# princeton-computational-imaging/Neural-Volume-Super-Resolution

Hardware: AMD Instinct MI355X
Metric: rendered rays/sec (64+128 samples) at 800x800 Lego-like view (higher is better)
Workload: dtype f32 as 2 f16 limbs (3 MFMA products, f32 acc); 1 GPU; Blender-'lego'-like 800x800 view, 64 coarse + 128 fine samples, tri-plane decoder (3x800^2x48 + 32^2x48 planes, 4+4x128 MLP), 1 view per GPU per step; partition=view

## Files before the change

include/nvsr.h:

```cpp
#ifndef NVSR_H
#define NVSR_H
#include <stdint.h>

#ifdef __cplusplus
extern "C" {
#endif

typedef void* nvsr_stream_t;

typedef enum {
    NVSR_OK = 0,
    NVSR_ERR_SHAPE = 1,
    NVSR_ERR_LAUNCH = 2,
    NVSR_ERR_NULL = 3,
    NVSR_ERR_ALIGN = 4
} nvsr_status;

#define NVSR_PLANE_CHANNELS 48
#define NVSR_DEC_CHANNELS 128
#define NVSR_DEC_LAYERS 4
#define NVSR_DECODER_NATURAL_FLOATS 130564
#define NVSR_DECODER_PACKED_F32_FLOATS 130576
#define NVSR_DECODER_PACKED_FLOATS 453136
#define NVSR_DECODER_PACKED_BWD_FLOATS 487424

typedef struct nvsr_scene {
    const float* planes[4];
    int32_t ph[4], pw[4];
    float lo[5];
    float range[5];
    float proj[3][6];
} nvsr_scene;

int nvsr_version(void);

#define NVSR_ARITH_INHERIT (-1)
#define NVSR_ARITH_INVALID (-2)
#define NVSR_ARITH_F32 0
#define NVSR_ARITH_F16X2 2
#define NVSR_ARITH_BF16X3 3
#define NVSR_ARITH_DEFAULT NVSR_ARITH_F16X2
int nvsr_get_decoder_arithmetic(void);
int nvsr_set_decoder_arithmetic(int mode);
int nvsr_set_range_flag(uint32_t* device_word);
uint32_t* nvsr_get_range_flag(void);
int nvsr_release_render_scratch(void);
int64_t nvsr_render_scratch_bytes(void);
int nvsr_internal_group_order(const int* trips, int64_t G, int S, int* out, nvsr_stream_t stream);
int nvsr_internal_copy_group_order(int* dst, int64_t G, nvsr_stream_t stream);
int nvsr_internal_live_order(int* live_n, int64_t N, int S, nvsr_stream_t stream);
int nvsr_internal_colour_order_bins(void);
int nvsr_internal_copy_live_counts(int* dst, int64_t N, nvsr_stream_t stream);
int nvsr_internal_point_order(const int* entries, const float* lists, const float* rays, int64_t N, int S, int bands, int* points, int* steps, int* offsets,
                              nvsr_stream_t stream);
int nvsr_internal_point_bands(void);
int nvsr_internal_copy_point_steps(int* dst, int64_t G, nvsr_stream_t stream);
int64_t nvsr_occupancy_words(int G);
int64_t nvsr_occupancy_workspace_floats(int G, int K);
int nvsr_occupancy_build(const nvsr_scene* scene, const float* packed_decoder, int G, int K, float threshold, int dilate, int arithmetic, uint32_t* grid,
                         float* workspace, nvsr_stream_t stream);
int nvsr_render_pass_occupancy_arith(const nvsr_scene* scene, const float* packed_decoder, int64_t N, int S, const float* rays, const float* z, int lindisp,
                                     int white_bkgd, float* rgb, float* disp, float* acc, float* weights, float* depth, const uint32_t* grid, int G, int arithmetic,
                                     nvsr_stream_t stream);
int nvsr_render_rays_occupancy_arith(const nvsr_scene* scene, const float* packed_coarse, const float* packed_fine, int64_t N, int Nc, int Nf,
                                     const float* rays, int lindisp, int white_bkgd, const float* t_rand, const float* u, float* rgb_c, float* disp_c,
                                     float* acc_c, float* rgb_f, float* disp_f, float* acc_f, float* workspace, const uint32_t* grid_coarse, int G_coarse,
                                     const uint32_t* grid_fine, int G_fine, int arithmetic, nvsr_stream_t stream);
int nvsr_internal_occupancy_probes(const nvsr_scene* scene, int G, int K, float* x, nvsr_stream_t stream);
int nvsr_internal_occupancy_cull(const nvsr_scene* scene, int64_t N, int S, const float* rays, const float* z, int lindisp, const uint32_t* grid, int G, int* kept,
                                 int* kept_n, nvsr_stream_t stream);
int nvsr_internal_copy_kept_counts(int* dst, int64_t N, nvsr_stream_t stream);
int nvsr_limb_gemm_probe(int arithmetic, int K, const float* W, const float* X, float* Y, nvsr_stream_t stream);
#define NVSR_CONV_ARITH_DEFAULT NVSR_ARITH_F16X2
int nvsr_get_conv_arithmetic(void);
int nvsr_set_conv_arithmetic(int mode);

int nvsr_plane_to_channel_last(const float* nchw, float* nhwc, int C, int H, int W, nvsr_stream_t stream);
int nvsr_plane_from_channel_last(const float* nhwc, float* nchw, int C, int H, int W, nvsr_stream_t stream);

int nvsr_pack_decoder(const float* natural, float* packed, nvsr_stream_t stream);

int nvsr_get_ray_bundle(int H, int W, double focal_x, double focal_y, const float* c2w, int padding, double offset,
                        float* ro, float* rd, nvsr_stream_t stream);
int nvsr_get_ray_bundle_at(int H, int W, double focal_x, double focal_y, const float* c2w, double offset, int64_t N, const int32_t* row_col,
                           float* ro, float* rd, nvsr_stream_t stream);
int nvsr_sample_pixels(int64_t total, int H, int W, uint64_t key, int64_t first, int64_t n, const float* image, int channels,
                       int32_t* row_col, float* target, nvsr_stream_t stream);
uint64_t nvsr_sample_key(uint64_t seed, uint64_t calls);
int nvsr_sample_pixels_seq(int64_t total, int H, int W, uint64_t* state, int64_t first, int64_t n, const float* image, int channels,
                           int32_t* row_col, float* target, nvsr_stream_t stream);
#define NVSR_MSE_PAIR_MAX_ELEMS (1 << 22)
int nvsr_mse_pair(int64_t n, const float* a, const float* b, const float* target, float* losses, float* g_a, float* g_b, nvsr_stream_t stream);
int nvsr_mse_pair_sum(int64_t n, const float* a, const float* b, const float* target, float* losses3, nvsr_stream_t stream);
int nvsr_mse_pair_backward(int64_t n, const float* a, const float* b, const float* target, const float* scale_a, const float* scale_b, float* g_a,
                           float* g_b, nvsr_stream_t stream);
int nvsr_ndc_rays(int H, int W, double focal, double near_, int64_t N, const float* ro, const float* rd, float* ro_out,
                  float* rd_out, nvsr_stream_t stream);
int nvsr_pack_rays(int64_t N, const float* ro, const float* rd, const float* view_src, double near_, double far_,
                   float* rays, nvsr_stream_t stream);
int nvsr_coarse_z(int64_t N, int Nc, const float* rays, int lindisp, const float* t_rand, float* z, nvsr_stream_t stream);

int nvsr_sample_pdf(int64_t N, int nb, int ns, const float* bins, const float* weights, const float* u, float* samples,
                    nvsr_stream_t stream);
int nvsr_cumprod_exclusive(int64_t N, int n, const float* in, float* out, nvsr_stream_t stream);
int nvsr_cumprod_exclusive_backward(int64_t N, int n, const float* in, const float* out, const float* g_out, float* g_in,
                                    nvsr_stream_t stream);
int nvsr_sort_rows(int64_t N, int n, const float* in, float* out, nvsr_stream_t stream);
int nvsr_importance_resample(int64_t N, int Nc, int Nf, const float* z_coarse, const float* weights, const float* u,
                             float* z_fine, nvsr_stream_t stream);

int nvsr_importance_resample_rays(int64_t N, int Nc, int Nf, const float* rays, int lindisp, const float* weights, const float* u,
                                  float* z_fine, nvsr_stream_t stream);

int nvsr_triplane_decode(const nvsr_scene* scene, const float* packed_decoder, int64_t P, const float* x, float* out,
                         nvsr_stream_t stream);
int nvsr_triplane_decode_arith(const nvsr_scene* scene, const float* packed_decoder, int64_t P, const float* x, float* out, int arithmetic,
                               nvsr_stream_t stream);

int nvsr_composite(int64_t N, int S, const float* raw, const float* z, const float* rd, const float* noise, int white_bkgd,
                   float* rgb, float* disp, float* acc, float* weights, float* depth, nvsr_stream_t stream);

int nvsr_composite_mip(int64_t N, int S, const float* raw, const float* z, const float* rd, const float* noise, int white_bkgd,
                       float* rgb, float* disp, float* acc, float* weights , float* depth ,
                       nvsr_stream_t stream);
int nvsr_composite_rays(int64_t N, int S, const float* raw, const float* z, const float* rays, const float* noise, int white_bkgd,
                        float* rgb, float* disp, float* acc, float* weights, float* depth, nvsr_stream_t stream);

int nvsr_render_pass(const nvsr_scene* scene, const float* packed_decoder, int64_t N, int S, const float* rays, const float* z,
                     const float* noise, int white_bkgd, float* rgb, float* disp, float* acc, float* weights, float* depth,
                     nvsr_stream_t stream);

int nvsr_decode_rays(const nvsr_scene* scene, const float* packed_decoder, int64_t N, int S, const float* rays, const float* z,
                     float* raw, nvsr_stream_t stream);

#define NVSR_FUSED_MIN_RAYS 65536
int64_t nvsr_fused_min_rays(void);
int64_t nvsr_render_workspace_floats(int64_t N, int Nc, int Nf);
int nvsr_render_rays(const nvsr_scene* scene, const float* packed_coarse, const float* packed_fine, int64_t N, int Nc, int Nf,
// ... 245 lines not shown
```

neural-volume-super-resolution_amd/capi.py:

```python
import ctypes as C
import os

import torch

from .build import LIB_PATH as _DEFAULT_LIB_PATH

LIB_PATH = os.environ.get("NVSR_HIP_LIB", _DEFAULT_LIB_PATH)

PLANE_CHANNELS = 48
DEC_CHANNELS = 128
DECODER_NATURAL_FLOATS = 130564
DECODER_PACKED_FLOATS = 453136
DECODER_PACKED_BWD_FLOATS = 487424
MIP_NERF_NATURAL_FLOATS = 81092
MIP_NERF_RECORD_FLOATS = 767
MIP_NERF_GRAD_RECORD_FLOATS = 708
PE_NERF_NATURAL_FLOATS = 81476
PE_NERF_RECORD_FLOATS = 770
PE_NERF_GRAD_RECORD_FLOATS = 708
MSE_PAIR_MAX_ELEMS = 1 << 22

_STATUS = {1: "NVSR_ERR_SHAPE (argument out of the supported range)", 2: "NVSR_ERR_LAUNCH (kernel launch failed)",
           3: "NVSR_ERR_NULL (required pointer is NULL)", 4: "NVSR_ERR_ALIGN (pointer not 16-byte aligned)"}

# ... 59 lines not shown
    "nvsr_cumprod_exclusive_backward": ([_i64, _i, _vp, _vp, _vp, _vp, _vp], _i),
    "nvsr_importance_resample": ([_i64, _i, _i, _vp, _vp, _vp, _vp, _vp], _i),
    "nvsr_importance_resample_rays": ([_i64, _i, _i, _vp, _i, _vp, _vp, _vp, _vp], _i),
    "nvsr_triplane_decode": ([C.POINTER(Scene), _vp, _i64, _vp, _vp, _vp], _i),
    "nvsr_triplane_decode_arith": ([C.POINTER(Scene), _vp, _i64, _vp, _vp, _i, _vp], _i),
    "nvsr_composite": ([_i64, _i, _vp, _vp, _vp, _vp, _i, _vp, _vp, _vp, _vp, _vp, _vp], _i),
    "nvsr_composite_rays": ([_i64, _i, _vp, _vp, _vp, _vp, _i, _vp, _vp, _vp, _vp, _vp, _vp], _i),
    "nvsr_composite_mip": ([_i64, _i, _vp, _vp, _vp, _vp, _i, _vp, _vp, _vp, _vp, _vp, _vp], _i),
    "nvsr_render_pass": ([C.POINTER(Scene), _vp, _i64, _i, _vp, _vp, _vp, _i, _vp, _vp, _vp, _vp, _vp, _vp], _i),
    "nvsr_decode_rays": ([C.POINTER(Scene), _vp, _i64, _i, _vp, _vp, _vp, _vp], _i),
    "nvsr_render_workspace_floats": ([_i64, _i, _i], _i64),
    "nvsr_render_rays": ([C.POINTER(Scene), _vp, _vp, _i64, _i, _i, _vp, _i, _i, _vp, _vp, _vp, _vp, _vp, _vp, _vp, _vp, _vp,
                          _vp, _vp, _vp], _i),
}
PACK_ALL_ARITHMETICS = -3
_fp = C.POINTER(C.c_float)
_ip = C.POINTER(C.c_int)
_PROTOS_OPTIONAL = {
    "nvsr_conv3x3_packed_floats": ([_i, _i], _i64),
    "nvsr_pack_conv3x3": ([_vp, _i, _i, _vp, _vp], _i),
    "nvsr_conv3x3": ([_vp, _i, _i, _i, _vp, _i, _i, _vp, _vp, _vp], _i),
    "nvsr_edsr_natural_floats": ([_i, _i, _i, _i, _i], _i64),
    "nvsr_edsr_packed_floats": ([_i, _i, _i, _i, _i], _i64),
    "nvsr_pack_edsr": ([_vp, _i, _i, _i, _i, _i, _vp, _vp], _i),
    "nvsr_pack_edsr_arith": ([_vp, _i, _i, _i, _i, _i, _vp, _i, _vp], _i),
    "nvsr_edsr_out_size": ([_i, _i, _i, _i, _ip, _ip], _i),
    "nvsr_edsr_workspace_floats": ([_i, _i, _i, _i, _i], _i64),
    "nvsr_edsr_forward": ([_vp, _i, _i, _i, _vp, _i, _i, _i, _i, _vp, _vp, _vp], _i),
    "nvsr_planes_sr_workspace_floats": ([_i, _i, _i, _i, _i, _i, _i, _fp], _i64),
    "nvsr_planes_sr": ([_vp, _i, _i, _i, _vp, _i, _i, _i, _i, _i, _fp, _vp, _vp, _vp, _vp, _vp], _i),
    "nvsr_render_pass_ex": ([C.POINTER(Scene), _vp, _i64, _i, _vp, _vp, _vp, _i, _vp, _vp, _vp, _vp, _vp, _vp, _vp], _i),
    "nvsr_pack_decoder_bwd": ([_vp, _vp, _vp], _i),
    "nvsr_composite_backward": ([_i64, _i, _vp, _vp, _vp, _vp, _i, _vp, _vp, _vp, _vp], _i),
    "nvsr_composite_backward_mip": ([_i64, _i, _vp, _vp, _vp, _vp, _i, _vp, _vp, _vp, _vp], _i),
    "nvsr_composite_backward_depth": ([_i64, _i, _vp, _vp, _vp, _vp, _i, _vp, _vp, _vp, _i, _vp, _vp], _i),
    "nvsr_composite_backward_rays": ([_i64, _i, _vp, _vp, _vp, _vp, _i, _vp, _vp, _vp, _i, _vp, _vp], _i),
    "nvsr_render_pass_backward": ([C.POINTER(Scene), _vp, _vp, _i64, _i, _vp, _vp, _vp, C.POINTER(C.c_void_p), _vp], _i),
    "nvsr_decode_rays_ex": ([C.POINTER(Scene), _vp, _i64, _i, _vp, _vp, _vp, _vp, _vp, _vp], _i),
    "nvsr_render_pass_backward_gates": ([C.POINTER(Scene), _vp, _vp, _i64, _i, _vp, _vp, _vp, _vp, C.POINTER(C.c_void_p), _vp, _vp, _vp], _i),
    "nvsr_view_grad_workspace_floats": ([_i64, _i], _i64),
    "nvsr_decoder_record_floats": ([_i64, _i], _i64),
    "nvsr_render_pass_backward_ex": ([C.POINTER(Scene), _vp, _vp, _i64, _i, _vp, _vp, _vp, C.POINTER(C.c_void_p), _vp, _vp, _vp], _i),
    "nvsr_decoder_weight_grad": ([_i64, _i, _vp, _vp, _vp], _i),
    "nvsr_edsr_forward_batch": ([_vp, _i, _i, _i, _i, _vp, _i, _i, _i, _i, _vp, _vp, _vp], _i),
    "nvsr_planes_sr_batch": ([C.POINTER(C.c_void_p), _i, _i, _i, _i, _vp, _i, _i, _i, _i, _i, _fp, _vp, _vp, C.POINTER(C.c_void_p), _vp, _vp], _i),
    "nvsr_pack_conv3x3_dgrad": ([_vp, _i, _i, _vp, _vp], _i),
    "nvsr_conv3x3_dgrad": ([_vp, _i, _i, _i, _vp, _i, _vp, _vp], _i),
    "nvsr_conv3x3_wgrad_workspace_floats": ([_i, _i, _i, _i], _i64),
    "nvsr_conv3x3_wgrad": ([_vp, _vp, _i, _i, _i, _i, C.c_float, _vp, _vp, _vp], _i),
    "nvsr_edsr_acts_floats": ([_i, _i, _i, _i, _i, _i, _i], _i64),
    "nvsr_edsr_forward_train": ([_vp, _i, _i, _i, _vp, _i, _i, _i, _i, _vp, _vp, _vp], _i),
    "nvsr_edsr_packed_dgrad_floats": ([_i, _i, _i, _i, _i], _i64),
    "nvsr_pack_edsr_dgrad": ([_vp, _i, _i, _i, _i, _i, _vp, _vp], _i),
    "nvsr_pack_edsr_dgrad_arith": ([_vp, _i, _i, _i, _i, _i, _vp, _i, _vp], _i),
    "nvsr_edsr_backward_workspace_floats": ([_i, _i, _i, _i, _i, _i, _i], _i64),
    "nvsr_edsr_backward": ([_vp, _i, _i, _i, _vp, _vp, _i, _i, _i, _i, _vp, _vp, _vp, _vp, _vp], _i),
    "nvsr_planes_sr_keep_floats": ([_i, _i, _i, _i, _i, _i, _i, _fp], _i64),
    "nvsr_planes_sr_train": ([_vp, _i, _i, _i, _vp, _i, _i, _i, _i, _i, _fp, _vp, _vp, _vp, _vp, _vp, _vp], _i),
    "nvsr_planes_sr_backward_workspace_floats": ([_i, _i, _i, _i, _i, _i, _i, _fp], _i64),
    "nvsr_planes_sr_backward": ([_i, _i, _i, _vp, _vp, _i, _i, _i, _i, _i, _fp, _vp, _vp, _vp, _vp, _vp, _vp], _i),
    "nvsr_generic_decoder_natural_floats": ([C.POINTER(DecoderGeometry)], _i64),
    "nvsr_generic_decode_workspace_floats": ([C.POINTER(DecoderGeometry), _i64], _i64),
    "nvsr_generic_decode": ([C.POINTER(Scene), C.POINTER(DecoderGeometry), _vp, _i64, _vp, _vp, _vp, _vp], _i),
    "nvsr_generic_decode_backward_workspace_floats": ([C.POINTER(DecoderGeometry), _i64], _i64),
    "nvsr_generic_decode_backward": ([C.POINTER(Scene), C.POINTER(DecoderGeometry), _vp, _i64, _vp, _vp, _vp, _vp, _vp, _vp, _vp, _vp, _vp], _i),
    "nvsr_generic_decoder_natural_floats_ext": ([C.POINTER(DecoderGeometry), _i], _i64),
    "nvsr_generic_decode_workspace_floats_ext": ([C.POINTER(DecoderGeometry), _i, _i64], _i64),
    "nvsr_generic_decode_backward_workspace_floats_ext": ([C.POINTER(DecoderGeometry), _i, _i64], _i64),
    "nvsr_generic_decode_ext": ([C.POINTER(SceneExt), C.POINTER(DecoderGeometry), _vp, _i64, _vp, _vp, _vp, _vp, _vp], _i),
    "nvsr_generic_decode_backward_ext": ([C.POINTER(SceneExt), C.POINTER(DecoderGeometry), _vp, _i64, _vp, _vp, _vp, _vp, C.POINTER(C.c_void_p),
                                          _vp, _vp], _i),
    "nvsr_ray_points": ([_i64, _i, _vp, _vp, _vp, _vp], _i),
    "nvsr_render_shared_workspace_floats": ([_i64, _i, _i], _i64),
    "nvsr_render_rays_shared_arith": ([C.POINTER(Scene), _vp, _i64, _i, _i, _vp, _i, _i, _vp, _vp, _vp, _vp, _vp, _vp, _vp, _vp, _vp, _vp, _vp, _i, _vp], _i),
    "nvsr_shared_merge": ([_i64, _i, _i, _vp, _i, _vp, _vp, _vp, _vp, _vp, _vp], _i),
    "nvsr_release_render_scratch": ([], _i),
    "nvsr_render_scratch_bytes": ([], _i64),
    "nvsr_internal_group_order": ([_vp, _i64, _i, _vp, _vp], _i),
    "nvsr_internal_copy_group_order": ([_vp, _i64, _vp], _i),
    "nvsr_internal_live_order": ([_vp, _i64, _i, _vp], _i),
    "nvsr_internal_colour_order_bins": ([], _i),
    "nvsr_internal_copy_live_counts": ([_vp, _i64, _vp], _i),
    "nvsr_internal_point_bands": ([], _i),
    "nvsr_internal_copy_point_steps": ([_vp, _i64, _vp], _i),
    "nvsr_internal_point_order": ([_vp, _vp, _vp, _i64, _i, _i, _vp, _vp, _vp, _vp], _i),
    "nvsr_occupancy_words": ([_i], _i64),
    "nvsr_occupancy_workspace_floats": ([_i, _i], _i64),
    "nvsr_occupancy_build": ([C.POINTER(Scene), _vp, _i, _i, C.c_float, _i, _i, _vp, _vp, _vp], _i),
    "nvsr_render_pass_occupancy_arith": ([C.POINTER(Scene), _vp, _i64, _i, _vp, _vp, _i, _i, _vp, _vp, _vp, _vp, _vp, _vp, _i, _i, _vp], _i),
    "nvsr_render_rays_occupancy_arith": ([C.POINTER(Scene), _vp, _vp, _i64, _i, _i, _vp, _i, _i, _vp, _vp, _vp, _vp, _vp, _vp, _vp, _vp, _vp, _vp, _i, _vp, _i,
                                          _i, _vp], _i),
    "nvsr_internal_occupancy_probes": ([C.POINTER(Scene), _i, _i, _vp, _vp], _i),
    "nvsr_internal_occupancy_cull": ([C.POINTER(Scene), _i64, _i, _vp, _vp, _i, _vp, _i, _vp, _vp, _vp], _i),
    "nvsr_internal_copy_kept_counts": ([_vp, _i64, _vp], _i),
    "nvsr_set_sr_plane_interp": ([_i], _i),
    "nvsr_get_sr_plane_interp": ([], _i),
    "nvsr_set_sr_align_corners": ([_i], _i),
    "nvsr_get_sr_align_corners": ([], _i),
    "nvsr_render_pass_arith": ([C.POINTER(Scene), _vp, _i64, _i, _vp, _vp, _vp, _i, _vp, _vp, _vp, _vp, _vp, _vp, _i, _vp], _i),
    "nvsr_decode_rays_arith": ([C.POINTER(Scene), _vp, _i64, _i, _vp, _vp, _vp, _vp, _vp, _i, _vp], _i),
    "nvsr_render_rays_arith": ([C.POINTER(Scene), _vp, _vp, _i64, _i, _i, _vp, _i, _i, _vp, _vp, _vp, _vp, _vp, _vp, _vp, _vp, _vp,
                                _vp, _vp, _i, _vp], _i),
    "nvsr_render_pass_backward_gates_arith": ([C.POINTER(Scene), _vp, _vp, _i64, _i, _vp, _vp, _vp, _vp, C.POINTER(C.c_void_p), _vp, _vp, _i, _vp], _i),
    "nvsr_decoder_weight_grad_arith": ([_i64, _i, _vp, _vp, _i, _vp], _i),
    "nvsr_conv3x3_arith": ([_vp, _i, _i, _i, _vp, _i, _i, _vp, _vp, _i, _i, _vp], _i),
    "nvsr_conv3x3_dgrad_arith": ([_vp, _i, _i, _i, _vp, _i, _vp, _i, _i, _vp], _i),
    "nvsr_conv3x3_wgrad_arith": ([_vp, _vp, _i, _i, _i, _i, C.c_float, _vp, _vp, _i, _vp], _i),
    "nvsr_edsr_forward_batch_arith": ([_vp, _i, _i, _i, _i, _vp, _i, _i, _i, _i, _vp, _vp, _i, _vp], _i),
    "nvsr_edsr_forward_train_arith": ([_vp, _i, _i, _i, _vp, _i, _i, _i, _i, _vp, _vp, _i, _vp], _i),
    "nvsr_edsr_backward_arith": ([_vp, _i, _i, _i, _vp, _vp, _i, _i, _i, _i, _vp, _vp, _vp, _vp, _i, _vp], _i),
    "nvsr_planes_sr_arith": ([_vp, _i, _i, _i, _vp, _i, _i, _i, _i, _i, _fp, _vp, _vp, _vp, _vp, _i, _vp], _i),
    "nvsr_planes_sr_batch_arith": ([C.POINTER(C.c_void_p), _i, _i, _i, _i, _vp, _i, _i, _i, _i, _i, _fp, _vp, _vp, C.POINTER(C.c_void_p), _vp, _i, _vp], _i),
    "nvsr_planes_sr_train_arith": ([_vp, _i, _i, _i, _vp, _i, _i, _i, _i, _i, _fp, _vp, _vp, _vp, _vp, _vp, _i, _vp], _i),
    "nvsr_planes_sr_backward_arith": ([_i, _i, _i, _vp, _vp, _i, _i, _i, _i, _i, _fp, _vp, _vp, _vp, _vp, _vp, _i, _vp], _i),
    "nvsr_planes_sr_batch_ex": ([C.POINTER(C.c_void_p), _i, _i, _i, _i, _vp, _i, _i, _i, _i, _i, _fp, _vp, _vp, C.POINTER(C.c_void_p), _vp, _i, _i, _i, _vp], _i),
    "nvsr_planes_sr_batch_keep_floats": ([_i, _i, _i, _i, _i, _i, _i, _i, _fp], _i64),
    "nvsr_planes_sr_batch_workspace_floats": ([_i, _i, _i, _i, _i, _i, _i, _i, _fp], _i64),
    "nvsr_planes_sr_batch_backward_workspace_floats": ([_i, _i, _i, _i, _i, _i, _i, _i, _fp], _i64),
    "nvsr_planes_sr_train_batch_arith": ([C.POINTER(C.c_void_p), _i, _i, _i, _i, _vp, _i, _i, _i, _i, _i, _fp, _vp, _vp, C.POINTER(C.c_void_p), _vp, _vp,
                                          _i, _i, _i, _vp], _i),
    "nvsr_planes_sr_backward_batch_arith": ([_i, _i, _i, _i, _vp, _vp, _i, _i, _i, _i, _i, _fp, _vp, C.POINTER(C.c_void_p), _vp, C.POINTER(C.c_void_p), _vp,
                                             _i, _i, _i, _vp], _i),
    "nvsr_planes_sr_backward_batch_marks": ([_i, _i, _i, _i, _vp, _vp, _i, _i, _i, _i, _i, _fp, _vp, C.POINTER(C.c_void_p), _vp, C.POINTER(C.c_void_p), _vp,
                                             _i, _i, _i, _i, C.POINTER(C.c_int32), C.POINTER(C.c_void_p), _vp], _i),
    "nvsr_positional_encoding": ([_i64, _i, _vp, _i, _i, _vp, _vp], _i),
    "nvsr_flexible_nerf_forward": ([_i64, _vp, _i, _i, _i, _i, _i, _vp, _vp, _vp], _i),
    "nvsr_mip_encode": ([_i64, _i, _vp, _vp, _d, _vp, _vp], _i),
    "nvsr_mip_nerf_forward_arith": ([_i64, _i, _vp, _vp, _d, _vp, _vp, _vp, _i, _vp], _i),
    "nvsr_mip_nerf_backward_arith": ([_i64, _vp, _vp, _vp, _vp, _i, _vp], _i),
    "nvsr_mip_nerf_wgrad_workspace_floats": ([_i64], _i64),
    "nvsr_mip_nerf_weight_grad": ([_i64, _vp, _vp, _vp, _vp, _vp], _i),
    "nvsr_pe_encode": ([_i64, _i, _vp, _vp, _vp, _vp], _i),
    "nvsr_pe_nerf_forward_arith": ([_i64, _i, _vp, _vp, _vp, _vp, _vp, _i, _vp], _i),
    "nvsr_pe_nerf_backward_arith": ([_i64, _vp, _vp, _vp, _vp, _i, _vp], _i),
    "nvsr_pe_nerf_wgrad_workspace_floats": ([_i64], _i64),
    "nvsr_pe_nerf_weight_grad": ([_i64, _vp, _vp, _vp, _vp, _vp], _i),
    "nvsr_render_pass_backward_rows_arith": ([C.POINTER(Scene), _vp, _vp, _i64, _i, _vp, _vp, _vp, _vp, C.POINTER(C.c_void_p), _vp, _vp, _i, _vp], _i),
    "nvsr_view_rows_reduce": ([_i64, _i, _vp, _vp, _vp], _i),
    "nvsr_internal_plane_taps": ([C.POINTER(Scene), _i, _i64, _i, _vp, _vp, _vp, _vp, _vp], _i),
    "nvsr_rows_scatter_workspace_bytes": ([_i64], _i64),
    "nvsr_rows_scatter": ([_i64, _vp, _vp, _vp, _i, _i, _vp, _vp, _i64, _vp], _i),
    "nvsr_decoder_weight_grad_det_workspace_floats": ([_i64, _i], _i64),
    "nvsr_decoder_weight_grad_det_arith": ([_i64, _i, _vp, _vp, _vp, _i, _vp], _i),
    "nvsr_lowrank_planes": ([LowrankPlanesArgs, _vp], _i),
    "nvsr_lowrank_planes_backward": ([LowrankPlanesArgs, _vp], _i),
}

_PROTOS_LAUNCH = {
    "nvsr_render_pass2_launch": ([C.POINTER(Scene), _vp, _i64, _i, _vp, _vp, _vp, _i, _vp, _vp, _vp, _vp, _vp, _vp, _vp], _i),
    "nvsr_render_pass3_launch": ([_i, C.POINTER(Scene), _vp, _i64, _i, _vp, _vp, _vp, _i, _vp, _vp, _vp, _vp, _vp, _vp, _vp], _i),
    "nvsr_render_pass3_coarse_z_launch": ([_i, C.POINTER(Scene), _vp, _i64, _i, _vp, _i, _vp, _i, _vp, _vp, _vp, _vp, _vp, _vp, _vp], _i),
    "nvsr_decode_rays_limb_launch": ([_i, C.POINTER(Scene), _vp, _i64, _i, _vp, _vp, _vp, _vp, _vp, _vp], _i),
    "nvsr_decode_rays_pair_launch": ([C.POINTER(Scene), _vp, _i64, _i, _vp, _vp, _vp, _vp, _vp], _i),
}

_lib = None


ARITHMETIC = {"f32": 0, "f16x2": 2, "bf16x3": 3}
SR_BATCH_MAX = 4
ARITH_INHERIT = -1


def arith_code(mode):
    if mode is None:
        return ARITH_INHERIT
# ... 169 lines not shown
```

neural-volume-super-resolution_amd/csrc/colour_order.hip:

```cpp
#include "colour_order.h"
#include "occupancy.h"
#include "nvsr_internal.h"

#include <cstdlib>
#include <mutex>
#include <vector>

namespace nvsr {

constexpr int SORT_TPB = 1024, SORT_WAVES = SORT_TPB / 64, SORT_ROUNDS = 4, SORT_MAX = SORT_TPB * SORT_ROUNDS;
template <int NKEYS>
__device__ __forceinline__ void counting_sort(const int (&key)[SORT_ROUNDS], int nkeys, int n, int (&start)[SORT_ROUNDS], int (&place)[SORT_ROUNDS],
                                              int (&len)[SORT_ROUNDS]) {
    static_assert(NKEYS <= SORT_TPB, "one thread per key sums the tables");
    __shared__ int cnt_s[NKEYS * SORT_WAVES];
    __shared__ int tot_s[NKEYS], start_s[NKEYS];
    const int wave = threadIdx.x >> 6, lane = threadIdx.x & 63;
    const unsigned long long below = (1ull << lane) - 1ull;
    for (int b = 0; b <= nkeys; ++b) {
        int c = 0;
#pragma unroll
        for (int r = 0; r < SORT_ROUNDS; ++r) c += __popcll(__ballot(key[r] == b));
        if (lane == 0) cnt_s[b * SORT_WAVES + wave] = c;
    }
    __syncthreads();
    if ((int)threadIdx.x <= nkeys) {
        int run = 0;
        for (int w = 0; w < SORT_WAVES; ++w) { const int c = cnt_s[threadIdx.x * SORT_WAVES + w]; cnt_s[threadIdx.x * SORT_WAVES + w] = run; run += c; }
        tot_s[threadIdx.x] = run;
    }
    __syncthreads();
    if ((int)threadIdx.x <= nkeys) {
        int run = 0;
        for (int b = nkeys; b > (int)threadIdx.x; --b) run += tot_s[b];
        start_s[threadIdx.x] = run;
    }
    __syncthreads();
#pragma unroll
    for (int r = 0; r < SORT_ROUNDS; ++r) start[r] = place[r] = len[r] = 0;
    if (wave * (64 * SORT_ROUNDS) >= n) return;
    for (int b = 0; b <= nkeys; ++b) {
        int at = cnt_s[b * SORT_WAVES + wave];
#pragma unroll
        for (int r = 0; r < SORT_ROUNDS; ++r) {
            const unsigned long long m = __ballot(key[r] == b);
            if (key[r] == b) place[r] = at + __popcll(m & below);
            at += __popcll(m);
        }
    }
#pragma unroll
    for (int r = 0; r < SORT_ROUNDS; ++r)
        if (key[r] >= 0) { start[r] = start_s[key[r]]; len[r] = tot_s[key[r]]; }
}

static_assert(ORDER_RAYS == SORT_MAX && SORT_WAVES == ORDER_RAYS / RAYS2 && RAYS2 % 64 == 0, "one block of the order per sort, one wave of it per colour workgroup");
__global__ __launch_bounds__(SORT_TPB) void live_order_kernel(int* __restrict__ live_n, long N, int S, int bins, int* __restrict__ group_trip) {
    __shared__ int out_s[ORDER_RAYS];
    const long block_base = (long)blockIdx.x * ORDER_RAYS;
    const int M = (int)(N - block_base < ORDER_RAYS ? N - block_base : ORDER_RAYS);
    const int wave = threadIdx.x >> 6, lane = threadIdx.x & 63;
    int cnt[SORT_ROUNDS], bin[SORT_ROUNDS];
#pragma unroll
    for (int r = 0; r < SORT_ROUNDS; ++r) {
        const int i = wave * (64 * SORT_ROUNDS) + r * 64 + lane;
        cnt[r] = i < M ? live_n[block_base + i] : 0;
        const int b = (int)(((unsigned)cnt[r] * (unsigned)bins + (unsigned)(S - 1)) / (unsigned)S);
        bin[r] = i < M ? (b < bins ? b : bins) : -1;
    }
    int start[SORT_ROUNDS], place[SORT_ROUNDS], len[SORT_ROUNDS];
    counting_sort<ORDER_BINS + 1>(bin, bins, M, start, place, len);
#pragma unroll
    for (int r = 0; r < SORT_ROUNDS; ++r)
        if (bin[r] >= 0) out_s[start[r] + place[r]] = (cnt[r] << ORDER_SHIFT) | (wave * (64 * SORT_ROUNDS) + r * 64 + lane);
    __syncthreads();
#pragma unroll
    for (int r = 0; r < SORT_ROUNDS; ++r) {
        const int i = threadIdx.x + r * SORT_TPB;
        if (i < M) live_n[block_base + i] = out_s[i];
    }
    if (group_trip && wave * RAYS2 < M) {
        int m = 0;
#pragma unroll
        for (int r = 0; r < RAYS2 / 64; ++r) {
            const int i = wave * RAYS2 + r * 64 + lane;
            if (i < M) m = max(m, out_s[i] >> ORDER_SHIFT);
        }
#pragma unroll
        for (int o = 32; o >= 1; o >>= 1) m = max(m, __shfl_xor(m, o));
        if (lane == 0) group_trip[(long)blockIdx.x * SORT_WAVES + wave] = m;
    }
}

constexpr int GORDER_MAX_G = SORT_MAX, GORDER_MAX_S = 511;
__global__ __launch_bounds__(SORT_TPB) void group_order_kernel(const int* __restrict__ group_trip, int G, int S, int sorted, int* __restrict__ group_slot) {
    if (!sorted || G > GORDER_MAX_G || S > GORDER_MAX_S) {
        const unsigned per = (unsigned)G >> 3, rem = (unsigned)G & 7u;
        for (unsigned r = threadIdx.x; r < (unsigned)G; r += SORT_TPB) {
            const unsigned xcd = r & 7u;
            group_slot[r] = (int)(xcd * per + (xcd < rem ? xcd : rem) + (r >> 3));
        }
        return;
    }
    const int wave = threadIdx.x >> 6, lane = threadIdx.x & 63;
    int key[SORT_ROUNDS];
#pragma unroll
    for (int r = 0; r < SORT_ROUNDS; ++r) {
        const int g = wave * (64 * SORT_ROUNDS) + r * 64 + lane;
        const int t = g < G ? group_trip[g] : 0;
        key[r] = g < G ? (t < 0 ? 0 : t > S ? S : t) : -1;
    }
    int start[SORT_ROUNDS], place[SORT_ROUNDS], len[SORT_ROUNDS];
    counting_sort<GORDER_MAX_S + 1>(key, S, G, start, place, len);
#pragma unroll
    for (int r = 0; r < SORT_ROUNDS; ++r) {
        if (key[r] < 0) continue;
        const int run = len[r], per = run >> 3, rem = run & 7, thr = rem * (per + 1);
        const int j = place[r];
        const int k = j < thr ? j / (per + 1) : rem + (j - thr) / (per ? per : 1);
        const int i = j < thr ? j - k * (per + 1) : (j - thr) - (k - rem) * per;
        group_slot[start[r] + k + 8 * i] = wave * (64 * SORT_ROUNDS) + r * 64 + lane;
    }
}

__global__ __launch_bounds__(RAYS2) void point_order_kernel(const int* __restrict__ live_n, const float* __restrict__ live_z, const float* __restrict__ rays_nf,
                                                            long N, int S, int nb, int* __restrict__ pts, int* __restrict__ steps, int* __restrict__ offs) {
    __shared__ int wsum_s[2][RAYS2 / 64], kmin_s[RAYS2], cnt_s[RAYS2], start_s[RAYS2], stage_s[RAYS2];
    const int j = threadIdx.x, wave = j >> 6, lane = j & 63;
    const long slot0 = (long)blockIdx.x * RAYS2;
    int n = 0;
    long ray = 0;
    if (slot0 + j < N) {
        const int e = live_n[slot0 + j];
        n = e >> ORDER_SHIFT;
        ray = slot0 / ORDER_RAYS * ORDER_RAYS + (e & (ORDER_RAYS - 1));
    }
    const float* lz = live_z + ray * S;
    const float nr = rays_nf ? rays_nf[ray * 11 + 6] : 0.0f, fr = rays_nf ? rays_nf[ray * 11 + 7] : 0.0f;
    auto band_of = [&](int k) -> int {
        const float e = lz[k];
        if (!rays_nf) {
            const long long b = (long long)__float_as_int(e) * nb / S;
            return b < 0 ? 0 : b < nb ? (int)b : nb - 1;
        }
        const float u = __fdiv_rn(__fmul_rn(__fsub_rn(e, nr), (float)nb), __fsub_rn(fr, nr));
        return u >= 0.0f ? (u < (float)nb ? (int)u : nb - 1) : 0;
    };
    auto scan = [&](int c, int buf, int& total) -> int {
        int incl = c;
#pragma unroll
        for (int o = 1; o < 64; o <<= 1) { const int v = __shfl_up(incl, o); if (lane >= o) incl += v; }
        if (lane == 63) wsum_s[buf][wave] = incl;
        __syncthreads();
        int before = 0;
        total = 0;
#pragma unroll
        for (int w = 0; w < RAYS2 / 64; ++w) { const int v = wsum_s[buf][w]; if (w < wave) before += v; total += v; }
        return before + incl - c;
    };
    int* out = pts + (long)blockIdx.x * RAYS2 * S;
    int k = 0, base = 0, nextb = n > 0 ? band_of(0) : nb;
    for (int b = 0; b < nb; ++b) {
        const int k0 = k;
        while (k < n && nextb <= b) { ++k; if (k < n) nextb = max(nextb, band_of(k)); }
        int total;
        const int at = base + scan(k - k0, b & 1, total);
        for (int i = k0; i < k; ++i) out[at + (i - k0)] = (j << 24) | i;
        base += total;
    }
    const int nsteps = (base + RAYS2 - 1) / RAYS2;
    if (base + j < nsteps * RAYS2) out[base + j] = POINT_NONE;
    if (j == 0) { steps[blockIdx.x] = nsteps; offs[blockIdx.x] = (int)blockIdx.x * S; }
    __syncthreads();
    for (int t = 0; t < nsteps; ++t) {
        const int e = out[t * RAYS2 + j];
        const bool valid = e != POINT_NONE;
        const int sl = (int)((unsigned)e >> 24), kk = e & 0xffffff;
        kmin_s[j] = 0x7fffffff; cnt_s[j] = 0;
        __syncthreads();
        if (valid) { atomicMin(&kmin_s[sl], kk); atomicAdd(&cnt_s[sl], 1); }
        __syncthreads();
        int total;
        start_s[j] = scan(cnt_s[j], 0, total);
        __syncthreads();
        stage_s[valid ? start_s[sl] + (kk - kmin_s[sl]) : j] = e;
        __syncthreads();
        out[t * RAYS2 + j] = stage_s[j];
    }
}

namespace {
enum { LISTS, GROUP, POINTS, VIEWS, KEPT, KEPT_GROUP, N_BUFFERS };
struct Buffer { void* p; size_t bytes; };
struct Launch { int64_t N; int* n; int* steps; int64_t kept_N; int* kept; };
struct Scratch { int device; hipStream_t stream; Buffer buf[N_BUFFERS]; Launch last; };
std::mutex g_live_mutex;
std::vector<Scratch> g_live;

Scratch* find_scratch(int device, hipStream_t stream) {
    for (Scratch& c : g_live)
        if (c.device == device && c.stream == stream) return &c;
    return nullptr;
}

bool grow(Scratch& e, int which, size_t bytes) {
    Buffer& b = e.buf[which];
    if (b.bytes >= bytes) return true;
    if (b.p) (void)hipFree(b.p);
    b = Buffer{};
    e.last = Launch{};
    void* p = nullptr;
    if (hipMalloc(&p, bytes) != hipSuccess) { (void)hipGetLastError(); return false; }
    b = Buffer{p, bytes};
    return true;
}

int64_t groups_of(int64_t N) { return (N + RAYS2 - 1) / RAYS2; }

template <class Pick>
int copy_left_behind(int* dst, int64_t ints, nvsr_stream_t stream, Pick pick) {
    if (!dst) return NVSR_ERR_NULL;
    int device = 0;
    if (hipGetDevice(&device) != hipSuccess) return NVSR_ERR_LAUNCH;
    const int* src = nullptr;
    {
        std::lock_guard<std::mutex> lock(g_live_mutex);
        const Scratch* c = find_scratch(device, (hipStream_t)stream);
        if (c) src = pick(*c);
    }
    if (!src) return NVSR_ERR_SHAPE;
    return hipMemcpyAsync(dst, src, (size_t)ints * sizeof(int), hipMemcpyDefault, (hipStream_t)stream) == hipSuccess ? NVSR_OK : NVSR_ERR_LAUNCH;
}

bool env_starts(const char* name, char c) {
    const char* e = getenv(name);
    return e && e[0] == c;
}
void launch_live_order(int* live_n, int64_t N, int S, int bins, int* group_trip, hipStream_t stream) {
    hipLaunchKernelGGL(live_order_kernel, dim3((unsigned)((N + ORDER_RAYS - 1) / ORDER_RAYS)), dim3(SORT_TPB), 0, stream, live_n, (long)N, S, bins, group_trip);
}
void launch_group_order(const int* group_trip, int64_t G, int S, int* group_slot, hipStream_t stream) {
    const int sorted = !env_starts("NVSR_COLOUR_GROUP_ORDER", '0');
    hipLaunchKernelGGL(group_order_kernel, dim3(1), dim3(SORT_TPB), 0, stream, group_trip, (int)G, S, sorted, group_slot);
}
void launch_point_order(const int* live_n, const float* live_z, const float* rays_nf, int64_t N, int S, int nb, int* pts, int* steps, int* offs, hipStream_t stream) {
    nb = nb < 1 || nb > S ? S : nb;
    hipLaunchKernelGGL(point_order_kernel, dim3((unsigned)groups_of(N)), dim3(RAYS2), 0, stream, live_n, live_z, rays_nf, (long)N, S, nb, pts, steps, offs);
}
}

PassRoute acquire_pass_scratch(int64_t N, int S, hipStream_t stream, bool raw_out, bool want_kept, bool launch, LiveLists& live, KeptLists& kept) {
    bool declines = raw_out || S < 1 || S >= ORDER_MAX_S || env_starts("NVSR_RENDER_ONE_PHASE", '1');
    if (!declines) {
        hipStreamCaptureStatus cap = hipStreamCaptureStatusNone;
        if (hipStreamIsCapturing(stream, &cap) != hipSuccess || cap != hipStreamCaptureStatusNone) { (void)hipGetLastError(); declines = true; }
    }
    if (declines && !want_kept) return PassRoute::Fused;
    int device = 0;
    if (hipGetDevice(&device) != hipSuccess) return PassRoute::Fused;
    const size_t rows = (size_t)N * (size_t)S, G = (size_t)groups_of(N);
    std::lock_guard<std::mutex> lock(g_live_mutex);
    Scratch* e = find_scratch(device, stream);
    if (e && want_kept) { e->last.kept_N = 0; e->last.kept = nullptr; }
    if (declines) return PassRoute::Fused;
    if (!e) {
        g_live.emplace_back();
        e = &g_live.back();
        e->device = device; e->stream = stream;
    }
    if (!grow(*e, GROUP, 2 * G * sizeof(int)) || !grow(*e, LISTS, (2 * rows + (size_t)N) * sizeof(float)) || !e->buf[LISTS].p) return PassRoute::Fused;
    live = LiveLists{};
    live.z = static_cast<float*>(e->buf[LISTS].p);
    live.w = live.z + rows;
    live.n = reinterpret_cast<int*>(live.w + rows);
    live.slot = static_cast<int*>(e->buf[GROUP].p);
    live.trip = live.slot + G;
    const size_t npts = G * RAYS2 * (size_t)S;
    if (!env_starts("NVSR_COLOUR_POINTS", '0') && G * (size_t)S <= 0x7fffffffu && grow(*e, POINTS, (npts + 2 * G) * sizeof(int)) &&
        grow(*e, VIEWS, G * RAYS2 * POINT_VIEW_FLOATS * sizeof(float))) {
        live.pts = static_cast<int*>(e->buf[POINTS].p);
        live.steps = live.pts + npts;
        live.views = static_cast<float*>(e->buf[VIEWS].p);
    }
    PassRoute route = PassRoute::TwoPhase;
    if (want_kept && grow(*e, KEPT_GROUP, 2 * G * sizeof(int)) && grow(*e, KEPT, (rows + (size_t)N) * sizeof(int))) {
        kept.idx = static_cast<int*>(e->buf[KEPT].p);
        kept.n = kept.idx + rows;
        kept.slot = static_cast<int*>(e->buf[KEPT_GROUP].p);
        kept.trip = kept.slot + G;
        route = PassRoute::Occupancy;
    }
    if (launch) e->last = route == PassRoute::Occupancy ? Launch{N, live.n, live.steps, N, kept.n} : Launch{N, live.n, live.steps, e->last.kept_N, e->last.kept};
    return route;
}

static void launch_orders(int* n, int* trip, int* slot, int64_t N, int S, hipStream_t stream) {
    launch_live_order(n, N, S, env_starts("NVSR_COLOUR_ORDER", '0') ? 0 : ORDER_BINS, trip, stream);
    launch_group_order(trip, groups_of(N), S, slot, stream);
}
void launch_kept_order(const KeptLists& kl, int64_t N, int S, hipStream_t stream) { launch_orders(kl.n, kl.trip, kl.slot, N, S, stream); }
void launch_colour_order(const LiveLists& ll, int64_t N, int S, hipStream_t stream) { launch_orders(ll.n, ll.trip, ll.slot, N, S, stream); }

void launch_point_order(const LiveLists& ll, const float* rays_nf, int64_t N, int S, hipStream_t stream) {
    launch_point_order(ll.n, ll.z, rays_nf, N, S, POINT_BANDS, ll.pts, ll.steps, ll.steps + groups_of(N), stream);
}

}

using namespace nvsr;

extern "C" int nvsr_internal_colour_order_bins(void) { return ORDER_BINS; }
extern "C" int nvsr_internal_live_order(int* live_n, int64_t N, int S, nvsr_stream_t stream) {
    if (!live_n) return NVSR_ERR_NULL;
    if (N < 1 || S < 1 || S >= ORDER_MAX_S || (N + ORDER_RAYS - 1) / ORDER_RAYS > 0x7fffffff) return NVSR_ERR_SHAPE;
    launch_live_order(live_n, N, S, ORDER_BINS, nullptr, (hipStream_t)stream);
    return NVSR_CHECK_LAUNCH();
}
extern "C" int nvsr_internal_copy_live_counts(int* dst, int64_t N, nvsr_stream_t stream) {
    return copy_left_behind(dst, N, stream, [N](const Scratch& c) { return c.last.N == N ? c.last.n : nullptr; });
}
extern "C" int nvsr_internal_group_order(const int* trips, int64_t G, int S, int* out, nvsr_stream_t stream) {
    if (!trips || !out) return NVSR_ERR_NULL;
    if (G < 1 || G > 0x7fffffff || S < 1 || S >= ORDER_MAX_S) return NVSR_ERR_SHAPE;
    launch_group_order(trips, G, S, out, (hipStream_t)stream);
    return NVSR_CHECK_LAUNCH();
}
extern "C" int nvsr_internal_copy_group_order(int* dst, int64_t G, nvsr_stream_t stream) {
    return copy_left_behind(dst, 2 * G, stream, [G](const Scratch& c) { return c.last.n && groups_of(c.last.N) == G ? static_cast<int*>(c.buf[GROUP].p) : nullptr; });
}

extern "C" int nvsr_internal_point_bands(void) { return POINT_BANDS; }
extern "C" int nvsr_internal_point_order(const int* entries, const float* lists, const float* rays, int64_t N, int S, int bands, int* points, int* steps, int* offsets,
                                         nvsr_stream_t stream) {
    if (!entries || !lists || !points || !steps || !offsets) return NVSR_ERR_NULL;
    const int64_t G = (N + RAYS2 - 1) / RAYS2;
    if (N < 1 || S < 1 || S >= ORDER_MAX_S || G * S > 0x7fffffff) return NVSR_ERR_SHAPE;
    launch_point_order(entries, lists, rays, N, S, bands, points, steps, offsets, (hipStream_t)stream);
    return NVSR_CHECK_LAUNCH();
}
extern "C" int nvsr_internal_copy_point_steps(int* dst, int64_t G, nvsr_stream_t stream) {
    return copy_left_behind(dst, G, stream, [G](const Scratch& c) { return c.last.n && groups_of(c.last.N) == G ? c.last.steps : nullptr; });
}

extern "C" int nvsr_internal_copy_kept_counts(int* dst, int64_t N, nvsr_stream_t stream) {
    return copy_left_behind(dst, N, stream, [N](const Scratch& c) { return c.last.kept_N == N ? c.last.kept : nullptr; });
}

extern "C" void nvsr_internal_reserve_render_scratch(int64_t N, int S, nvsr_stream_t stream) {
    LiveLists live;
    KeptLists kept;
    (void)acquire_pass_scratch(N, S, (hipStream_t)stream,  false,  false,  false, live, kept);
}

extern "C" int64_t nvsr_render_scratch_bytes(void) {
    std::lock_guard<std::mutex> lock(g_live_mutex);
    int64_t total = 0;
    for (const Scratch& c : g_live) total += (int64_t)c.buf[LISTS].bytes;
    return total;
}

extern "C" int nvsr_release_render_scratch(void) {
    std::lock_guard<std::mutex> lock(g_live_mutex);
    int prev = 0;
    const bool have_prev = hipGetDevice(&prev) == hipSuccess;
    int rc = NVSR_OK;
    for (const Scratch& c : g_live)
        for (const Buffer& b : c.buf)
            if (b.p && (hipSetDevice(c.device) != hipSuccess || hipFree(b.p) != hipSuccess)) rc = NVSR_ERR_LAUNCH;
    g_live.clear();
    if (have_prev) (void)hipSetDevice(prev);
    return rc;
}
```

Baseline: 8.121 million rays/s.

## Replace looped point-order kernel with single-pass bitmap and band-table counting-sort kernel

Adds a new point_order_kernel for S up to 256. It records each ray's per-band membership in a shared-memory bitmap, builds a per-band, per-wave count table with atomics, and scans it with DPP wave prefix sums. Each thread then places its points directly into 256-wide output steps, reading live_z as float4 when aligned. The old iterative kernel stays as a fallback for larger S. This aims to cut the repeated per-step passes and synchronisations of the loop kernel, but adds complex shared-memory bookkeeping and a larger shared footprint.

New measurement: 8.178 million rays/s (median of 6 runs). About the same (+0.7%).

```diff
diff --git a/include/nvsr.h b/include/nvsr.h
--- a/include/nvsr.h
+++ b/include/nvsr.h
@@ -54,6 +54,7 @@
 int nvsr_internal_point_order(const int* entries, const float* lists, const float* rays, int64_t N, int S, int bands, int* points, int* steps, int* offsets,
                               nvsr_stream_t stream);
 int nvsr_internal_point_bands(void);
+int nvsr_internal_point_order_max_s(void);
 int nvsr_internal_copy_point_steps(int* dst, int64_t G, nvsr_stream_t stream);
 int64_t nvsr_occupancy_words(int G);
 int64_t nvsr_occupancy_workspace_floats(int G, int K);
diff --git a/neural-volume-super-resolution_amd/capi.py b/neural-volume-super-resolution_amd/capi.py
--- a/neural-volume-super-resolution_amd/capi.py
+++ b/neural-volume-super-resolution_amd/capi.py
@@ -165,6 +165,7 @@
     "nvsr_internal_colour_order_bins": ([], _i),
     "nvsr_internal_copy_live_counts": ([_vp, _i64, _vp], _i),
     "nvsr_internal_point_bands": ([], _i),
+    "nvsr_internal_point_order_max_s": ([], _i),
     "nvsr_internal_copy_point_steps": ([_vp, _i64, _vp], _i),
     "nvsr_internal_point_order": ([_vp, _vp, _vp, _i64, _i, _i, _vp, _vp, _vp, _vp], _i),
     "nvsr_occupancy_words": ([_i], _i64),
diff --git a/neural-volume-super-resolution_amd/csrc/colour_order.hip b/neural-volume-super-resolution_amd/csrc/colour_order.hip
--- a/neural-volume-super-resolution_amd/csrc/colour_order.hip
+++ b/neural-volume-super-resolution_amd/csrc/colour_order.hip
@@ -1,7 +1,9 @@
 #include "colour_order.h"
 #include "occupancy.h"
 #include "nvsr_internal.h"
-
+#include "wave_scan.h"
+
+#include <cstdint>
 #include <cstdlib>
 #include <mutex>
 #include <vector>
@@ -122,7 +124,161 @@
     }
 }
 
+constexpr int POINT_ORDER_MAX_S = RAYS2, POINT_ORDER_WORDS = 2 * POINT_ORDER_MAX_S / 32 + 1;
+static_assert(RAYS2 == 256 && POINT_ORDER_MAX_S <= RAYS2 && 64 * POINT_ORDER_MAX_S < (1 << 16), "four waves; one thread per band scans the table");
+
+__device__ __forceinline__ int wave_scan_add_int(int v) {
+    v += __builtin_amdgcn_update_dpp(0, v, DPP_ROW_SHR1, 0xf, 0xf, false);
+    v += __builtin_amdgcn_update_dpp(0, v, DPP_ROW_SHR2, 0xf, 0xf, false);
+    v += __builtin_amdgcn_update_dpp(0, v, DPP_ROW_SHR4, 0xf, 0xf, false);
+    v += __builtin_amdgcn_update_dpp(0, v, DPP_ROW_SHR8, 0xf, 0xf, false);
+    v += __builtin_amdgcn_update_dpp(0, v, DPP_ROW_BCAST15, 0xa, 0xf, false);
+    v += __builtin_amdgcn_update_dpp(0, v, DPP_ROW_BCAST31, 0xc, 0xf, false);
+    return v;
+}
+
+template <bool VEC>
 __global__ __launch_bounds__(RAYS2) void point_order_kernel(const int* __restrict__ live_n, const float* __restrict__ live_z, const float* __restrict__ rays_nf,
+                                                            long N, int S, int nb, int* __restrict__ pts, int* __restrict__ steps, int* __restrict__ offs) {
+    __shared__ int tab_s[POINT_ORDER_MAX_S * 4 + 1], wsum_s[4];
+    __shared__ unsigned bits_s[POINT_ORDER_WORDS * RAYS2];
+    NVSR_RACE_PROBE_DELAY(bits_s);
+    const int j = threadIdx.x, wave = j >> 6, lane = j & 63;
+    const long slot0 = (long)blockIdx.x * RAYS2;
+    int n = 0;
+    long ray = 0;
+    if (slot0 + j < N) {
+        const int e = live_n[slot0 + j];
+        n = min(e >> ORDER_SHIFT, S);
+        ray = slot0 / ORDER_RAYS * ORDER_RAYS + (e & (ORDER_RAYS - 1));
+    }
+    const float* lz = live_z + ray * S;
+    const float nr = rays_nf ? rays_nf[ray * 11 + 6] : 0.0f, fr = rays_nf ? rays_nf[ray * 11 + 7] : 0.0f;
+    auto band_of = [&](float e) -> int {
+        if (!rays_nf) {
+            const long long b = (long long)__float_as_int(e) * nb / S;
+            return b < 0 ? 0 : b < nb ? (int)b : nb - 1;
+        }
+        const float u = __fdiv_rn(__fmul_rn(__fsub_rn(e, nr), (float)nb), __fsub_rn(fr, nr));
+        return u >= 0.0f ? (u < (float)nb ? (int)u : nb - 1) : 0;
+    };
+    float c0 = 0.0f, c1 = 0.0f, c2 = 0.0f, c3 = 0.0f;
+    float4 nxt = make_float4(0.0f, 0.0f, 0.0f, 0.0f);
+    if (VEC && n > 0) nxt = *reinterpret_cast<const float4*>(lz);
+    auto entry = [&](int k) -> float {
+        if (!VEC) return lz[k];
+        if ((k & 3) == 0) {
+            c0 = nxt.x; c1 = nxt.y; c2 = nxt.z; c3 = nxt.w;
+            if (k + 4 < n) nxt = *reinterpret_cast<const float4*>(lz + k + 4);
+        }
+        const float e = c0;
+        c0 = c1; c1 = c2; c2 = c3;
+        return e;
+    };
+    if (j < nb) {
+#pragma unroll
+        for (int i = 0; i < 4; ++i) tab_s[j * 4 + i] = 0;
+    }
+    __syncthreads();
+    {
+        unsigned w = 0;
+        int p = 0;
+        auto skip = [&](int d) {
+            const int q = p + d;
+            while ((q >> 5) > (p >> 5)) { bits_s[(p >> 5) * RAYS2 + j] = w; w = 0; p = (p | 31) + 1; }
+            p = q;
+        };
+        int band = 0, run = 0;
+        for (int k = 0; k < n; ++k) {
+            const int b = max(band, band_of(entry(k)));
+            if (b != band) {
+                if (run) atomicAdd(&tab_s[band * 4 + wave], run);
+                skip(b - band);
+                band = b; run = 0;
+            }
+            w |= 1u << (p & 31);
+            skip(1);
+            ++run;
+        }
+        if (run) atomicAdd(&tab_s[band * 4 + wave], run);
+        skip(nb - band);
+        if (p & 31) bits_s[(p >> 5) * RAYS2 + j] = w;
+    }
+    __syncthreads();
+    int total;
+    {
+        int v[4] = {0, 0, 0, 0};
+        if (j < nb) {
+#pragma unroll
+            for (int i = 0; i < 4; ++i) v[i] = tab_s[j * 4 + i];
+        }
+        const int s = v[0] + v[1] + v[2] + v[3];
+        const int incl = wave_scan_add_int(s);
+        if (lane == 63) wsum_s[wave] = incl;
+        __syncthreads();
+        int before = 0;
+        total = 0;
+#pragma unroll
+        for (int i = 0; i < 4; ++i) { const int x = wsum_s[i]; if (i < wave) before += x; total += x; }
+        int at = before + incl - s;
+        if (j < nb) {
+#pragma unroll
+            for (int i = 0; i < 4; ++i) { tab_s[j * 4 + i] = at; at += v[i]; }
+        }
+        if (j == 0) tab_s[nb * 4] = total;
+        __syncthreads();
+    }
+    int* out = pts + (long)blockIdx.x * RAYS2 * S;
+    const unsigned tag = (unsigned)j << 24;
+    {
+        unsigned w = bits_s[j];
+        int p = 0, k = 0;
+        int t = 0, Q = 0, kmin = 0, cnt = 0;
+        auto count = [&]() -> int {
+            int c = 0;
+            for (;;) {
+                const int avail = 32 - (p & 31);
+                const int ones = __builtin_ctzll(~(unsigned long long)(w >> (p & 31)));
+                if (ones < avail) {
+                    c += ones; p += ones + 1;
+                    if ((p & 31) == 0) w = bits_s[(p >> 5) * RAYS2 + j];
+                    return c;
+                }
+                c += avail; p += avail;
+                w = bits_s[(p >> 5) * RAYS2 + j];
+            }
+        };
+        auto place = [&](int b, int c, int incl) {
+            const int lo = tab_s[b * 4], hi = tab_s[b * 4 + 4], mine = tab_s[b * 4 + wave] + incl - c;
+            const int k0 = k;
+            k += c;
+            if (hi == lo) return;
+            for (;;) {
+                const int T0 = t * RAYS2, E = T0 + RAYS2;
+                Q += max(0, min(mine, E) - max(lo, T0));
+                const int a = max(mine, T0), z = min(mine + c, E);
+                if (z > a) { if (cnt == 0) kmin = k0 + (a - mine); cnt += z - a; }
+                if (hi < E) break;
+                for (int i = 0; i < cnt; ++i) out[T0 + Q + i] = (int)(tag | (unsigned)(kmin + i));
+                ++t; Q = 0; cnt = 0;
+                if (hi == E) break;
+            }
+        };
+        for (int b = 0; b < nb; b += 2) {
+            const bool two = b + 1 < nb;
+            const int ca = count(), cb = two ? count() : 0;
+            const int incl = wave_scan_add_int(ca | (cb << 16));
+            place(b, ca, incl & 0xffff);
+            if (two) place(b + 1, cb, incl >> 16);
+        }
+        for (int i = 0; i < cnt; ++i) out[t * RAYS2 + Q + i] = (int)(tag | (unsigned)(kmin + i));
+    }
+    const int nsteps = (total + RAYS2 - 1) / RAYS2;
+    if (total + j < nsteps * RAYS2) out[total + j] = POINT_NONE;
+    if (j == 0) { steps[blockIdx.x] = nsteps; offs[blockIdx.x] = (int)blockIdx.x * S; }
+}
+
+__global__ __launch_bounds__(RAYS2) void point_order_loop_kernel(const int* __restrict__ live_n, const float* __restrict__ live_z, const float* __restrict__ rays_nf,
                                                             long N, int S, int nb, int* __restrict__ pts, int* __restrict__ steps, int* __restrict__ offs) {
     __shared__ int wsum_s[2][RAYS2 / 64], kmin_s[RAYS2], cnt_s[RAYS2], start_s[RAYS2], stage_s[RAYS2];
     const int j = threadIdx.x, wave = j >> 6, lane = j & 63;
@@ -244,7 +400,13 @@
 }
 void launch_point_order(const int* live_n, const float* live_z, const float* rays_nf, int64_t N, int S, int nb, int* pts, int* steps, int* offs, hipStream_t stream) {
     nb = nb < 1 || nb > S ? S : nb;
-    hipLaunchKernelGGL(point_order_kernel, dim3((unsigned)groups_of(N)), dim3(RAYS2), 0, stream, live_n, live_z, rays_nf, (long)N, S, nb, pts, steps, offs);
+    const dim3 grid((unsigned)groups_of(N)), block(RAYS2);
+    if (S > POINT_ORDER_MAX_S)
+        hipLaunchKernelGGL(point_order_loop_kernel, grid, block, 0, stream, live_n, live_z, rays_nf, (long)N, S, nb, pts, steps, offs);
+    else if (S % 4 == 0 && reinterpret_cast<uintptr_t>(live_z) % 16 == 0)
+        hipLaunchKernelGGL(point_order_kernel<true>, grid, block, 0, stream, live_n, live_z, rays_nf, (long)N, S, nb, pts, steps, offs);
+    else
+        hipLaunchKernelGGL(point_order_kernel<false>, grid, block, 0, stream, live_n, live_z, rays_nf, (long)N, S, nb, pts, steps, offs);
 }
 }
 
@@ -329,6 +491,7 @@
 }
 
 extern "C" int nvsr_internal_point_bands(void) { return POINT_BANDS; }
+extern "C" int nvsr_internal_point_order_max_s(void) { return POINT_ORDER_MAX_S; }
 extern "C" int nvsr_internal_point_order(const int* entries, const float* lists, const float* rays, int64_t N, int S, int bands, int* points, int* steps, int* offsets,
                                          nvsr_stream_t stream) {
     if (!entries || !lists || !points || !steps || !offsets) return NVSR_ERR_NULL;
```
